# Lainshower/debiasing-multi-modal

Measured on AMD Instinct MI355X. Metric: images/sec (embed+adapter step), CLIP-RN50 224px bs=1024, higher is better.
Workload: dtype f32; 1 GPU; CLIP-RN50 224px encode_image + adapter(1024-128-1024) CE/SGD step, 1024 images/GPU, global batch 1024 (the metric's configuration, CLIP-RN50 224px bs=1024 on one GPU); global_batch=1024, batch_per_gpu=1024, parallelism=dp1, collective=none

## Files before the change

### debiasing-multi-modal_amd/csrc/conv_patch.hip

```cpp
#include <stdlib.h>
#include "common.h"

namespace {

constexpr int TR = 4, TC = 28;
constexpr int PR = TR + 2, PC = TC + 2, PPX = PR * PC;
constexpr int CIN = 32, KTOT = 9 * CIN;
constexpr int WROW = KTOT + 8;

struct PatchP {
    const float* x; const float* x_absmax;
    const u16* w; int w_exp; const float* sc; const float* bias;
    float* y; float* y_absmax;
    int B, H, W, tiles_w, tiles_h, n_tiles;
};

__device__ __forceinline__ int pswz(int row) { return (row >> 2) & 3; }

template <int N, int POOL>
__global__ __launch_bounds__(256, N == 32 ? 3 : 2) void conv3x3_c32_kernel(const PatchP p) {
    constexpr int TN = N / 32, NLD = (PPX * 8 + 255) / 256;
    constexpr int PCL = POOL ? 40 : PC, PLN = PR * PCL * 32;
    __shared__ __attribute__((aligned(16))) u16 lds[N * WROW + 2 * PLN];
    u16* Wl = lds;
    u16* Pl = lds + N * WROW;
    const int tid = threadIdx.x, lane = tid & 63, wave = tid >> 6;
    const int fr = lane & 31, fh = lane >> 5;

    for (int i = tid; i < N * (KTOT / 8); i += 256) {
        const int n = i / (KTOT / 8), c = i - n * (KTOT / 8);
        *(u32x4*)(Wl + n * WROW + c * 8) = *(const u32x4*)(p.w + (size_t)n * KTOT + c * 8);
    }
    const int s_a = scale_exp(*p.x_absmax);
    const float a_sc = pow2f(s_a), acc_scale = pow2f(-s_a - p.w_exp);
    float sv[TN], bv[TN];
#pragma unroll
    for (int j = 0; j < TN; ++j) { sv[j] = p.sc[j * 32 + fr] * acc_scale; bv[j] = p.bias[j * 32 + fr]; }

    const int ml = wave * 32 + fr;
    int a_dy, a_c;
    bool a_ok;
    if (POOL) { const int o = ml >> 2, q = ml & 3; a_dy = 2 * (o / 14) + (q >> 1); a_c = 2 * (o % 14) + (q & 1); a_ok = ml < TR * TC; }
    else { a_dy = wave; a_c = fr; a_ok = fr < TC; }
    const int a_row0 = a_ok ? a_dy * PCL + a_c : 0;

    const long long img_bytes = (long long)p.H * p.W * CIN * 4;
    f32x4 pre[NLD];
    auto tile_coords = [&](int tile, int& b, int& h0, int& w0) {
        const int tw = tile % p.tiles_w, r = tile / p.tiles_w;
        b = r / p.tiles_h; h0 = (r - b * p.tiles_h) * TR; w0 = tw * TC;
    };
    auto load_patch = [&](int tile) {
        int b, h0, w0;
        tile_coords(tile, b, h0, w0);
        const __amdgpu_buffer_rsrc_t rs = desc(p.x, (long long)p.B * img_bytes, (long long)b * img_bytes);
#pragma unroll
        for (int k = 0; k < NLD; ++k) {
            const int idx = tid + 256 * k, i = idx >> 3, quad = idx & 7;
            const int py = i / PC, px = i - py * PC, h = h0 - 1 + py, w = w0 - 1 + px;
            const bool ok = i < PPX && h >= 0 && h < p.H && w >= 0 && w < p.W;
            pre[k] = __builtin_bit_cast(f32x4, __builtin_amdgcn_raw_buffer_load_b128(
                rs, ok ? (unsigned)((h * p.W + w) * (CIN * 4) + quad * 16) : OOR, 0, 0));
        }
    };
    auto store_patch = [&]() {
#pragma unroll
        for (int k = 0; k < NLD; ++k) {
            const int idx = tid + 256 * k, i = idx >> 3, quad = idx & 7;
            if (i < PPX) {
                unsigned hp[2], lp[2];
#pragma unroll
                for (int j = 0; j < 2; ++j) split2h_pair(pre[k][2 * j], pre[k][2 * j + 1], a_sc, hp[j], lp[j]);
                const int py = i / PC, row = py * PCL + (i - py * PC);
                const int off = row * 32 + (((quad >> 1) ^ pswz(row)) << 3) + ((quad & 1) << 2);
                *(u32x2*)(Pl + off) = (u32x2){hp[0], hp[1]};
                *(u32x2*)(Pl + PLN + off) = (u32x2){lp[0], lp[1]};
            }
        }
    };

    float amax = 0.f;
    int tile = blockIdx.x;
    if (tile < p.n_tiles) load_patch(tile);
    for (; tile < p.n_tiles; tile += gridDim.x) {
        store_patch();
        __syncthreads();
        if (tile + (int)gridDim.x < p.n_tiles) load_patch(tile + gridDim.x);

        f32x16 acc[TN];
#pragma unroll
        for (int j = 0; j < TN; ++j)
#pragma unroll
            for (int r = 0; r < 16; ++r) acc[j][r] = 0.f;
#pragma unroll
        for (int tap = 0; tap < 9; ++tap) {
            const int row = a_row0 + (tap / 3) * PCL + (tap % 3);
#pragma unroll
            for (int ks = 0; ks < 2; ++ks) {
                const int aoff = row * 32 + (((2 * ks + fh) ^ pswz(row)) << 3);
                const u32x4 ah = *(const u32x4*)(Pl + aoff), al = *(const u32x4*)(Pl + PLN + aoff);
                u32x4 wf[TN];
#pragma unroll
                for (int j = 0; j < TN; ++j) wf[j] = *(const u32x4*)(Wl + (j * 32 + fr) * WROW + tap * 32 + (2 * ks + fh) * 8);
#pragma unroll
                for (int j = 0; j < TN; ++j)
                    acc[j] = __builtin_amdgcn_mfma_f32_32x32x16_f16(__builtin_bit_cast(f16x8, al), __builtin_bit_cast(f16x8, wf[j]), acc[j], 0, 0, 0);
#pragma unroll
                for (int j = 0; j < TN; ++j)
                    acc[j] = __builtin_amdgcn_mfma_f32_32x32x16_f16(__builtin_bit_cast(f16x8, ah), __builtin_bit_cast(f16x8, wf[j]), acc[j], 0, 0, 0);
            }
        }
        int b, h0, w0;
        tile_coords(tile, b, h0, w0);
        if constexpr (POOL) {
            const int Hp = p.H >> 1, Wp = p.W >> 1;
            const long long tot = (long long)p.B * Hp * Wp * N * 4;
            const long long base_px = ((long long)b * Hp + (h0 >> 1)) * Wp + (w0 >> 1);
            const __amdgpu_buffer_rsrc_t rs = desc(p.y, tot, base_px * N * 4);
#pragma unroll
            for (int t = 0; t < 4; ++t) {
                const int o = wave * 8 + 2 * t + fh;
                const unsigned off = o < 28 ? (unsigned)(((o / 14) * Wp + (o % 14)) * (N * 4) + fr * 4) : OOR;
#pragma unroll
                for (int j = 0; j < TN; ++j) {
                    float v[4];
#pragma unroll
                    for (int q = 0; q < 4; ++q) v[q] = fmaxf(fmaf(acc[j][4 * t + q], sv[j], bv[j]), 0.f);
                    const float s = (((v[0] + v[1]) + v[2]) + v[3]) * 0.25f;
                    __builtin_amdgcn_raw_buffer_store_b32(__builtin_bit_cast(unsigned, s), rs, off, (unsigned)(j * 128), 0);
                    if (o < 28) amax = fmaxf(amax, fmaxf(fmaxf(v[0], v[1]), fmaxf(v[2], v[3])));
                }
            }
        } else {
            const long long tot = (long long)p.B * p.H * p.W * N * 4;
            const long long base_px = ((long long)b * p.H + h0) * p.W + w0;
            const __amdgpu_buffer_rsrc_t rs = desc(p.y, tot, base_px * N * 4);
#pragma unroll
            for (int r = 0; r < 16; ++r) {
                const int c = (r & 3) + 8 * (r >> 2) + 4 * fh, dy = wave;
                const bool m_ok = c < TC;
                const unsigned off = m_ok ? (unsigned)((dy * p.W + c) * (N * 4) + fr * 4) : OOR;
#pragma unroll
                for (int j = 0; j < TN; ++j) {
                    const float v = fmaxf(fmaf(acc[j][r], sv[j], bv[j]), 0.f);
                    __builtin_amdgcn_raw_buffer_store_b32(__builtin_bit_cast(unsigned, v), rs, off, (unsigned)(j * 128), 0);
                    if (m_ok) amax = fmaxf(amax, v);
                }
            }
        }
        __syncthreads();
    }
    if (p.y_absmax) {
        amax = wave_max(amax);
        float* red = (float*)Pl;
        if (lane == 0) red[wave] = amax;
        __syncthreads();
        if (tid == 0) {
            const float m = fmaxf(fmaxf(red[0], red[1]), fmaxf(red[2], red[3]));
            if (m > *(volatile const float*)p.y_absmax) atomicMax((unsigned*)p.y_absmax, __float_as_uint(m));
        }
    }
}

}

extern "C" int dbmm_conv3x3_c32_bn_relu_x2(const float* x, const float* x_absmax, const void* w_plane_f16, int w_exp,
                                           const float* scale, const float* bias, float* y, float* y_absmax, int64_t B, int64_t H,
                                           int64_t W, int64_t Cin, int64_t Cout, int pool, void* stream) {
    if (!x || !x_absmax || !w_plane_f16 || !scale || !bias || !y) return DBMM_E_ARG;
    if (B <= 0 || H <= 0 || W <= 0 || (pool != 0 && pool != 2)) return DBMM_E_SHAPE;
    if (Cin != CIN || (Cout != 32 && Cout != 64) || (H % TR) || (W % TC) || w_exp < -40 || w_exp > 40) return DBMM_E_UNSUPPORTED;
    if (H * W * CIN * 4 >= EXT_LIM || B * (H / TR) * (W / TC) > INT32_MAX) return DBMM_E_UNSUPPORTED;
    if (!dbmm_aligned16(x) || !dbmm_aligned16(w_plane_f16) || !dbmm_aligned16(y)) return DBMM_E_ALIGN;
    PatchP p{};
    p.x = x; p.x_absmax = x_absmax; p.w = (const u16*)w_plane_f16; p.w_exp = w_exp; p.sc = scale; p.bias = bias;
    p.y = y; p.y_absmax = y_absmax; p.B = (int)B; p.H = (int)H; p.W = (int)W;
    p.tiles_w = (int)(W / TC); p.tiles_h = (int)(H / TR); p.n_tiles = (int)(B * p.tiles_h * p.tiles_w);
    const int per_cu = Cout == 32 ? 3 : 2;
    const int grid = p.n_tiles < DBMM_N_CU * per_cu ? p.n_tiles : DBMM_N_CU * per_cu;
    hipStream_t s = (hipStream_t)stream;
    if (Cout == 32) {
        if (pool) hipLaunchKernelGGL((conv3x3_c32_kernel<32, 1>), dim3(grid), dim3(256), 0, s, p);
        else hipLaunchKernelGGL((conv3x3_c32_kernel<32, 0>), dim3(grid), dim3(256), 0, s, p);
    } else {
        if (pool) hipLaunchKernelGGL((conv3x3_c32_kernel<64, 1>), dim3(grid), dim3(256), 0, s, p);
        else hipLaunchKernelGGL((conv3x3_c32_kernel<64, 0>), dim3(grid), dim3(256), 0, s, p);
    }
    DBMM_CHECK_LAUNCH();
    return DBMM_OK;
}
```

Baseline: 37570 images/sec.

## Software-pipeline LDS fragment reads and keep leading weight fragments in registers

The conv3x3 MFMA inner loop becomes 18 flattened steps. LDS reads for activation and weight fragments are issued two steps ahead, and sched_barrier fences stop the compiler from reordering them, so LDS latency overlaps with MFMA work. The first few weight fragments (4 or 8 steps, depending on N) are loaded into registers once per block and reused across tiles, which removes repeated LDS reads. The extra fragment buffers and resident weights raise VGPR pressure, which could lower occupancy below the launch-bounds target or cause spills.

```diff
diff --git a/debiasing-multi-modal_amd/csrc/conv_patch.hip b/debiasing-multi-modal_amd/csrc/conv_patch.hip
--- a/debiasing-multi-modal_amd/csrc/conv_patch.hip
+++ b/debiasing-multi-modal_amd/csrc/conv_patch.hip
@@ -20,6 +20,9 @@
 template <int N, int POOL>
 __global__ __launch_bounds__(256, N == 32 ? 3 : 2) void conv3x3_c32_kernel(const PatchP p) {
     constexpr int TN = N / 32, NLD = (PPX * 8 + 255) / 256;
+    constexpr int NSTEP = 18, AHEAD = 2;
+    struct Frag { u32x4 ah, al, wf[TN]; };
+    constexpr int RW = N == 64 ? 8 : 4;
     constexpr int PCL = POOL ? 40 : PC, PLN = PR * PCL * 32;
     __shared__ __attribute__((aligned(16))) u16 lds[N * WROW + 2 * PLN];
     u16* Wl = lds;
@@ -80,35 +83,50 @@
     };
 
     float amax = 0.f;
+    u32x4 wres[RW][TN];
+    bool w_held = false;
     int tile = blockIdx.x;
     if (tile < p.n_tiles) load_patch(tile);
     for (; tile < p.n_tiles; tile += gridDim.x) {
         store_patch();
         __syncthreads();
         if (tile + (int)gridDim.x < p.n_tiles) load_patch(tile + gridDim.x);
+        if (!w_held) {
+#pragma unroll
+            for (int s = 0; s < RW; ++s)
+#pragma unroll
+                for (int j = 0; j < TN; ++j) wres[s][j] = *(const u32x4*)(Wl + (j * 32 + fr) * WROW + (s >> 1) * 32 + (2 * (s & 1) + fh) * 8);
+            w_held = true;
+        }
 
         f32x16 acc[TN];
 #pragma unroll
         for (int j = 0; j < TN; ++j)
 #pragma unroll
             for (int r = 0; r < 16; ++r) acc[j][r] = 0.f;
-#pragma unroll
-        for (int tap = 0; tap < 9; ++tap) {
+        auto read_frag = [&](int s, Frag& f) {
+            const int tap = s >> 1, ks = s & 1;
             const int row = a_row0 + (tap / 3) * PCL + (tap % 3);
-#pragma unroll
-            for (int ks = 0; ks < 2; ++ks) {
-                const int aoff = row * 32 + (((2 * ks + fh) ^ pswz(row)) << 3);
-                const u32x4 ah = *(const u32x4*)(Pl + aoff), al = *(const u32x4*)(Pl + PLN + aoff);
-                u32x4 wf[TN];
-#pragma unroll
-                for (int j = 0; j < TN; ++j) wf[j] = *(const u32x4*)(Wl + (j * 32 + fr) * WROW + tap * 32 + (2 * ks + fh) * 8);
-#pragma unroll
-                for (int j = 0; j < TN; ++j)
-                    acc[j] = __builtin_amdgcn_mfma_f32_32x32x16_f16(__builtin_bit_cast(f16x8, al), __builtin_bit_cast(f16x8, wf[j]), acc[j], 0, 0, 0);
-#pragma unroll
-                for (int j = 0; j < TN; ++j)
-                    acc[j] = __builtin_amdgcn_mfma_f32_32x32x16_f16(__builtin_bit_cast(f16x8, ah), __builtin_bit_cast(f16x8, wf[j]), acc[j], 0, 0, 0);
-            }
+            const int aoff = row * 32 + (((2 * ks + fh) ^ pswz(row)) << 3);
+            f.ah = *(const u32x4*)(Pl + aoff); f.al = *(const u32x4*)(Pl + PLN + aoff);
+#pragma unroll
+            for (int j = 0; j < TN; ++j) f.wf[j] = s < RW ? wres[s][j] : *(const u32x4*)(Wl + (j * 32 + fr) * WROW + tap * 32 + (2 * ks + fh) * 8);
+        };
+        Frag fs[AHEAD + 1];
+#pragma unroll
+        for (int s = 0; s < AHEAD; ++s) read_frag(s, fs[s]);
+#pragma unroll
+        for (int s = 0; s < NSTEP; ++s) {
+            if (s + AHEAD < NSTEP) read_frag(s + AHEAD, fs[(s + AHEAD) % (AHEAD + 1)]);
+            __builtin_amdgcn_sched_barrier(0);
+            const Frag& f = fs[s % (AHEAD + 1)];
+#pragma unroll
+            for (int j = 0; j < TN; ++j)
+                acc[j] = __builtin_amdgcn_mfma_f32_32x32x16_f16(__builtin_bit_cast(f16x8, f.al), __builtin_bit_cast(f16x8, f.wf[j]), acc[j], 0, 0, 0);
+#pragma unroll
+            for (int j = 0; j < TN; ++j)
+                acc[j] = __builtin_amdgcn_mfma_f32_32x32x16_f16(__builtin_bit_cast(f16x8, f.ah), __builtin_bit_cast(f16x8, f.wf[j]), acc[j], 0, 0, 0);
+            __builtin_amdgcn_sched_barrier(0);
         }
         int b, h0, w0;
         tile_coords(tile, b, h0, w0);
```

Result: no change. 37590 images/sec, median of 2 (+0.0%).
